# submission2019/cnn-quantization

Measured on NVIDIA H100. Metric: resnet50_w4a4_images_per_s, higher is better.
Workload: dtype f32

## Files before the change

cnn-quantization_b200/csrc/fq_cl.cuh:

```cuda
#pragma once

namespace fqb {

__device__ __forceinline__ unsigned enc_ordered(float x) {
  const unsigned b = __float_as_uint(x);
  return (b & 0x80000000u) ? ~b : (b | 0x80000000u);
}
__device__ __forceinline__ float dec_ordered(unsigned e) {
  return __uint_as_float((e & 0x80000000u) ? (e & 0x7fffffffu) : ~e);
}

constexpr unsigned kAccU = 2u * kMaxNhwcChannels;
constexpr unsigned kAccD = 3u * kMaxNhwcChannels;

struct ClView {
  unsigned* amin_inv;
  unsigned* amax;
  double* asum;
  double* asq;
  double* aabs;
};
__device__ __forceinline__ ClView cl_view(const FusedArgs& A, unsigned bank) {
  ClView v;
  v.amin_inv = A.amin_inv + bank * kAccU;
// ... 313 lines not shown
  T* st = reinterpret_cast<T*>(buf);
  consumer_sync();
#pragma unroll
  for (int i = 0; i < 4; ++i) st[i * kConsumers + threadIdx.x] = (threadIdx.x < stride) ? v[i] : identity;
  consumer_sync();
#pragma unroll
  for (unsigned k = 0; k < kClItems; ++k) {
    const unsigned it = threadIdx.x + k * kConsumers;
    T a = identity;
    if (it < 4u * cv) {
      const unsigned col = it % cv, i = it / cv;
      for (unsigned t = col; t < stride; t += cv) a = op(a, st[i * kConsumers + t]);
    }
    res[k] = a;
  }
}

__device__ __noinline__ void cl_combine_s1(unsigned char* buf, unsigned cv, unsigned stride, const unsigned (&umn)[4],
                                           const unsigned (&umx)[4], const double (&s)[4], const double (&q)[4], unsigned* dmn,
                                           unsigned* dmx, double* ds, double* dq) {
  if (cv == stride) {
    if (threadIdx.x < stride) {
#pragma unroll
      for (int i = 0; i < 4; ++i) {
        const unsigned c = 4u * threadIdx.x + i;
        red_max_u32(dmn + c, umn[i]);
        red_max_u32(dmx + c, umx[i]);
        red_add_f64(ds + c, s[i]);
        red_add_f64(dq + c, q[i]);
      }
    }
    return;
  }
  uint2 mm[4], rmm[kClItems];
#pragma unroll
  for (int i = 0; i < 4; ++i) mm[i] = make_uint2(umn[i], umx[i]);
  auto max2 = [](uint2 a, uint2 b) { return make_uint2(a.x > b.x ? a.x : b.x, a.y > b.y ? a.y : b.y); };
  double rs[kClItems], rq[kClItems];
  cl_stage_round(buf, cv, stride, mm, make_uint2(0u, 0u), max2, rmm);
  cl_stage_round(buf, cv, stride, s, 0.0, OpAdd(), rs);
  cl_stage_round(buf, cv, stride, q, 0.0, OpAdd(), rq);
#pragma unroll
  for (unsigned k = 0; k < kClItems; ++k) {
    const unsigned it = threadIdx.x + k * kConsumers;
    if (it < 4u * cv) {
      const unsigned c = 4u * (it % cv) + it / cv;
      red_max_u32(dmn + c, rmm[k].x);
      red_max_u32(dmx + c, rmm[k].y);
      red_add_f64(ds + c, rs[k]);
      red_add_f64(dq + c, rq[k]);
    }
  }
}
__device__ __noinline__ void cl_combine_add_f64(unsigned char* buf, unsigned cv, unsigned stride, const double (&v0)[4], double* d0,
                                                const double (&v1)[4], double* d1, const double (&v2)[4], double* d2) {
  if (cv == stride) {
    if (threadIdx.x < stride) {
#pragma unroll
      for (int i = 0; i < 4; ++i) {
        const unsigned c = 4u * threadIdx.x + i;
        red_add_f64(d0 + c, v0[i]);
        if (d1) red_add_f64(d1 + c, v1[i]);
        if (d2) red_add_f64(d2 + c, v2[i]);
      }
    }
    return;
  }
  double r0[kClItems], r1[kClItems], r2[kClItems];
  cl_stage_round(buf, cv, stride, v0, 0.0, OpAdd(), r0);
  if (d1) cl_stage_round(buf, cv, stride, v1, 0.0, OpAdd(), r1);
  if (d2) cl_stage_round(buf, cv, stride, v2, 0.0, OpAdd(), r2);
#pragma unroll
  for (unsigned k = 0; k < kClItems; ++k) {
    const unsigned it = threadIdx.x + k * kConsumers;
    if (it < 4u * cv) {
      const unsigned c = 4u * (it % cv) + it / cv;
      red_add_f64(d0 + c, r0[k]);
      if (d1) red_add_f64(d1 + c, r1[k]);
      if (d2) red_add_f64(d2 + c, r2[k]);
    }
  }
}

template <typename T, typename Op>
__device__ __forceinline__ T cl_rep_reduce(const T* p, unsigned rep, unsigned C, unsigned c, T identity, Op op) {
  T v[8];
#pragma unroll
  for (unsigned r = 0; r < 8u; ++r) v[r] = (r < rep) ? ld_ws(p + r * C + c) : identity;
  return op(op(op(v[0], v[1]), op(v[2], v[3])), op(op(v[4], v[5]), op(v[6], v[7])));
}
__device__ __forceinline__ double cl_mean(const ClView& acc, unsigned rep, unsigned C, unsigned c, float k, float bias, double n) {
  const double s = cl_rep_reduce(acc.asum, rep, C, c, 0.0, OpAdd());
  return static_cast<double>(k) + static_cast<double>(bias) + s / n;
}
__device__ __forceinline__ float cl_std(const ClView& acc, unsigned rep, unsigned C, unsigned c, double n) {
  const double s = cl_rep_reduce(acc.asum, rep, C, c, 0.0, OpAdd());
  const double q = cl_rep_reduce(acc.asq, rep, C, c, 0.0, OpAdd());
  double m2 = q - s * s / n;
  if (m2 < 0.0) m2 = 0.0;
  return static_cast<float>(sqrt(m2 / (n - 1.0)));
}

__device__ __forceinline__ LeafParam mid_tread_param(const FusedArgs& A, float omega, float mn, float mx, float mu, float b,
                                                     float& rng) {
  const bool sym = !A.positive;
  if (A.mt_clip) {
    double om = sym ? static_cast<double>(omega) : 2.0 * static_cast<double>(omega);
    int i = 0;
    while (i < kTable - 1 && kOmegaTable[i] < om) ++i;
    double am;
    if (i == 0) {
      am = kAlphaTable[0];
    } else {
      const double inc = (kAlphaTable[i] - kAlphaTable[i - 1]) / (kOmegaTable[i] - kOmegaTable[i - 1]);
      am = kAlphaTable[i] - inc * (kOmegaTable[i] - om);
    }
    const float amf = static_cast<float>(am);
    rng = sym ? __fmul_rn(__fmul_rn(2.f, amf), b) : __fadd_rn(fmaxf(mu, 0.f), __fmul_rn(amf, b));
  } else {
    rng = sym ? __fsub_rn(mx, mn) : mx;
  }
  const float step = (omega > 0.f) ? __fdiv_rn(rng, omega) : 3.402823466e+38f;
  LeafParam q;
  q.a = step;
  q.flags = 0;
  if (A.mt_clip) {
    const float mu_q = sym ? __fdiv_rn(mu, step) : __fdiv_rn(fmaxf(mu, 0.f), step);
    q.c = __fadd_rn(mu_q, sym ? __fmul_rn(omega, 0.5f) : omega);
    q.b = sym ? __fsub_rn(mu_q, __fmul_rn(omega, 0.5f)) : 0.f;
  } else {
    q.b = -INFINITY;
    q.c = INFINITY;
  }
  return q;
}

__device__ __noinline__ void cl_solve_aux(const FusedArgs& A, const ClView& acc, LeaderSmem& sm, unsigned tag, bool have_b,
                                          bool publish) {
  const unsigned C = A.flat.channels;
  const double n = A.n_per_group;
  const bool prior_b = (A.leaf != FQB200_LEAF_MIDTREAD) && A.prior == FQB200_PRIOR_B;
  for (unsigned c = threadIdx.x; c < C; c += kConsumers) {
    if (prior_b) {
      const double sa = have_b ? cl_rep_reduce(acc.aabs, A.nhwc_rep, C, c, 0.0, OpAdd()) : 0.0;
      A.gb[c] = static_cast<float>(sa / n);
    } else {
      A.gstd[c] = cl_std(acc, A.nhwc_rep, C, c, n);
    }
  }
  consumer_sync();
  stamp(A, 10);
  if (A.leaf == FQB200_LEAF_MIDTREAD) {
    double local = 0.0;
    for (unsigned c = threadIdx.x; c < C; c += kConsumers) {
      const float p = powf(A.gstd[c], 0.6666666666666666f);
      A.gprior[c] = p;
      local += static_cast<double>(p);
    }
    const float psum = static_cast<float>(block_reduce(local, OpAdd(), sm.d));
    const float budget = static_cast<float>(static_cast<double>(C) * exp2(static_cast<double>(A.mt_target)));
    for (unsigned c = threadIdx.x; c < C; c += kConsumers) A.gbits[c] = rintf(__fdiv_rn(__fmul_rn(budget, A.gprior[c]), psum));
  } else {
    solve_bit_alloc(A, sm);
  }
  consumer_sync();
  if (publish && threadIdx.x == 0) st_release_u32(&A.sync->aux_ready, tag);
}

template <int LEAF, bool DEV>
__device__ __noinline__ LeafParam cl_channel_param(const FusedArgs& A, const ClView& acc, unsigned rep, unsigned C, unsigned c,
                                                   float mu, double n, bool alloc, bool do_export) {
  auto umax = [](unsigned a, unsigned b) { return a > b ? a : b; };
  const unsigned lo = cl_rep_reduce(acc.amin_inv, rep, C, c, 0u, umax);
  const unsigned hi = cl_rep_reduce(acc.amax, rep, C, c, 0u, umax);
  const double sa = DEV ? cl_rep_reduce(acc.aabs, rep, C, c, 0.0, OpAdd()) : 0.0;
  const float cb = A.bias ? __ldg(A.bias + c) : 0.f;
  const float mn = __fadd_rn(dec_ordered(~lo), cb), mx = __fadd_rn(dec_ordered(hi), cb);
  const float b = DEV ? static_cast<float>(sa / n) : 0.f;
  const bool need_sd = A.range_mode == FQB200_RANGE_GAUS || A.range_mode == FQB200_RANGE_KSTD || do_export;
  const float sd = need_sd ? cl_std(acc, rep, C, c, n) : 0.f;
  const float aux = alloc ? ld_ws(A.gbits + c) : static_cast<float>(A.num_bits);
  LeafParam q;
  if constexpr (LEAF == FQB200_LEAF_MIDTREAD) {
    float rng;
    q = mid_tread_param(A, aux, mn, mx, mu, b, rng);
    if (do_export) export_stats(A, c, mn, mx, mu, b, sd, rng, 0.f, aux, q);
  } else {
    float delta, offset;
    solve_range(A, mn, mx, mu, b, sd, aux, delta, offset);
    q = make_leaf_param(LEAF, delta, offset, aux);
    if (do_export) export_stats(A, c, mn, mx, mu, b, sd, delta, offset, aux, q);
  }
  return q;
}

struct ClCtx {
  const FlatGeo* g;
  BulkRing* ring;
  unsigned char* stages;
  unsigned char* cbuf;
  RingPos pos;
  ClView acc;
  unsigned rep_base, c0;
  bool active;
};

__device__ __noinline__ void cl_phase_s1(const FusedArgs& A, ClCtx& cx, float (&kshift)[4]) {
  const FlatGeo& g = *cx.g;
  ClStats1 s1;
  s1.init(A, cx.c0, cx.active);
#pragma unroll
  for (int i = 0; i < 4; ++i) kshift[i] = s1.k[i];
  RingPos pos = cx.pos;
  consume_phase(g, *cx.ring, cx.stages, pos, s1);
  cx.pos = pos;
  s1.flush();
  if (blockIdx.x == 0) stamp(A, 13);
  unsigned umn[4], umx[4];
#pragma unroll
  for (int i = 0; i < 4; ++i) {
    umn[i] = ~enc_ordered(s1.mn[i]);
    umx[i] = enc_ordered(s1.mx[i]);
  }
  const ClView& acc = cx.acc;
  const unsigned rb = cx.rep_base;
  cl_combine_s1(cx.cbuf, g.cv, g.stride, umn, umx, s1.s, s1.q, acc.amin_inv + rb, acc.amax + rb, acc.asum + rb, acc.asq + rb);
}

__device__ __noinline__ void cl_phase_s2(const FusedArgs& A, ClCtx& cx, const float (&mean)[4]) {
  const FlatGeo& g = *cx.g;
  ClStats2 s2;
  s2.init(A, cx.c0, cx.active, mean);
  RingPos pos = cx.pos;
  consume_phase(g, *cx.ring, cx.stages, pos, s2);
  cx.pos = pos;
  s2.flush();
  if (blockIdx.x == 0) stamp(A, 14);
  const ClView& acc = cx.acc;
  const unsigned rb = cx.rep_base;
  cl_combine_add_f64(cx.cbuf, g.cv, g.stride, s2.sa, acc.aabs + rb, s2.sa, nullptr, s2.sa, nullptr);
}

template <int LEAF, bool HIST>
__device__ __noinline__ void cl_phase_apply(const FusedArgs& A, ClCtx& cx, const LeafParam (&lp)[4], unsigned* hist) {
  const FlatGeo& g = *cx.g;
  const unsigned t = threadIdx.x;
  if (HIST) {
    for (unsigned i = t; i < kHistWords; i += kConsumers) hist[i] = 0u;
    consumer_sync();
  }
  ClApply<LEAF, HIST> ap{A, hist};
  ap.init(cx.c0, cx.active, lp);
  RingPos pos = cx.pos;
  if (A.pool.tiles) {
    if (A.pool.kind == 3u)
      consume_pool3_phase(g, A.pool, *cx.ring, cx.stages, pos, ap);
    else
      consume_pool_phase(g, A.pool, *cx.ring, cx.stages, pos, ap);
  } else if (A.residual) {
    const FlatGeo h = half_geo(g);
    consume_pair_phase(h, *cx.ring, cx.stages, pos, ap);
  } else {
    consume_phase(g, *cx.ring, cx.stages, pos, ap);
  }
  cx.pos = pos;
  if (HIST) {
    consumer_sync();
    const unsigned bins = static_cast<unsigned>(A.hist_bins);
    const unsigned copies = max(1u, min(static_cast<unsigned>(kWarps), kHistWords / bins));
    for (unsigned b = t; b < bins; b += kConsumers) {
      unsigned long long cnt = 0;
      for (unsigned w = 0; w < copies; ++w) cnt += hist[w * bins + b];
      if (cnt) atomicAdd(A.hist + b, cnt);
    }
    if (LEAF == FQB200_LEAF_MIDTREAD && A.hist_clamped && cx.active) {
#pragma unroll
// ... 20 lines not shown
  __shared__ LeaderSmem lsm;
  __shared__ alignas(8) unsigned long long solver_done;
  const FlatGeo& g = A.flat;
  const unsigned C = g.channels, cv = g.cv;
  const unsigned launch = ld_ws(&A.sync->launch_count);
  const unsigned bank = launch & 1u;
  const unsigned tag = launch + 1u;
  const bool alloc = (LEAF == FQB200_LEAF_MIDTREAD) || (A.bit_alloc && A.num_bits <= 4);
  const bool aux_needs_b = alloc && LEAF != FQB200_LEAF_MIDTREAD && A.prior == FQB200_PRIOR_B;
  const bool solver_in_s2 = alloc && !aux_needs_b && DEV && gridDim.x > 1u;
  __shared__ alignas(8) unsigned long long phase_go[2];
  if (threadIdx.x == 0) {
    mbar_init(smem_u32(&solver_done), 1u);
    mbar_init(smem_u32(&phase_go[0]), 1u);
    mbar_init(smem_u32(&phase_go[1]), 1u);
  }
  const unsigned nstages = HIST ? kStages - 1u : kStages;
  ring_init(ring, nstages);

  if (threadIdx.x >= kConsumers) {
    if (threadIdx.x == kConsumers) {
      RingPos pos;
      pos.init(nstages);
      const float4* src = reinterpret_cast<const float4*>(A.in);
      const TicketPlan all = {2u, blockIdx.x, gridDim.x, 2u * gridDim.x};
      const TicketPlan no0 = {blockIdx.x == 0 ? 0u : 2u, blockIdx.x - 1u, gridDim.x - 1u, 2u * (gridDim.x - 1u)};
      produce_phase<false>(g, src, &A.sync->unit_counter[0], all, ring, stages, pos);
      if (DEV) {
        mbar_wait(smem_u32(&phase_go[0]), 0u);
        if (solver_in_s2 && blockIdx.x == 0) mbar_wait(smem_u32(&solver_done), 0u);
        produce_phase<true>(g, src, &A.sync->unit_counter[1], solver_in_s2 ? no0 : all, ring, stages, pos);
      }
      if (!A.stats_only) {
        mbar_wait(smem_u32(&phase_go[1]), 0u);
        if (A.pool.tiles && A.pool.kind == 3u)
          produce_pool3_phase(g, A.pool, src, &A.sync->unit_counter[2], all, ring, stages, pos);
        else if (A.pool.tiles)
          produce_pool_phase(g, A.pool, src, &A.sync->unit_counter[2], all, ring, stages, pos);
        else if (A.residual)
          produce_phase<!DEV, true>(half_geo(g), src, &A.sync->unit_counter[2], all, ring, stages, pos,
                                    reinterpret_cast<const float4*>(A.residual));
        else
          produce_phase<!DEV>(g, src, &A.sync->unit_counter[2], all, ring, stages, pos);
      }
    }
    return;
  }

  const unsigned t = threadIdx.x;
  const bool active = t < g.stride;
  const bool direct = cv == g.stride;
  const unsigned col = active ? t % cv : 0u;
  const unsigned c0 = 4u * col;
  const double n = A.n_per_group;
  const ClView acc = cl_view(A, bank);
  const unsigned rep = A.nhwc_rep;
  const unsigned rep_base = (blockIdx.x % rep) * C;
  unsigned epoch = 0;
  if (blockIdx.x == 0) stamp(A, 0);

  if (blockIdx.x == gridDim.x - 1u) {
    const ClView other = cl_view(A, bank ^ 1u);
    uint4* zu = reinterpret_cast<uint4*>(other.amin_inv);
    uint4* zd = reinterpret_cast<uint4*>(other.asum);
    const uint4 z = make_uint4(0u, 0u, 0u, 0u);
    for (unsigned i = t; i < kAccU / 4u; i += kConsumers) zu[i] = z;
    for (unsigned i = t; i < kAccD / 2u; i += kConsumers) zd[i] = z;
  }

  ClCtx cx;
  cx.g = &g;
  cx.ring = &ring;
  cx.stages = stages;
  cx.cbuf = cbuf;
  cx.pos.init(nstages);
  cx.acc = acc;
  cx.rep_base = rep_base;
  cx.c0 = c0;
  cx.active = active;
  float kshift[4];
  cl_phase_s1(A, cx, kshift);
  if (t == 0) mbar_arrive(smem_u32(&phase_go[DEV ? 0 : 1]));
  if (blockIdx.x == 0) stamp(A, 1);
  grid_barrier_cl(A.sync, epoch);
  if (blockIdx.x == 0) stamp(A, 4);

  float mean[4];
  if (direct) {
#pragma unroll
    for (int i = 0; i < 4; ++i)
      mean[i] = static_cast<float>(cl_mean(acc, rep, C, c0 + i, kshift[i], (A.bias && active) ? __ldg(A.bias + c0 + i) : 0.f, n));
  } else {
    for (unsigned c = t; c < C; c += kConsumers)
      tab_mean[c] = static_cast<float>(cl_mean(acc, rep, C, c, ld_tensor(A.in + c), A.bias ? __ldg(A.bias + c) : 0.f, n));
    consumer_sync();
#pragma unroll
    for (int i = 0; i < 4; ++i) mean[i] = tab_mean[c0 + i];
  }

  if (alloc && !aux_needs_b && blockIdx.x == 0) {
    cl_solve_aux(A, acc, lsm, tag, false, !solver_in_s2);
    stamp(A, 12);
    if (t == 0) mbar_arrive(smem_u32(&solver_done));
  }

  if constexpr (DEV) {
    cl_phase_s2(A, cx, mean);
    if (t == 0) mbar_arrive(smem_u32(&phase_go[1]));
    if (blockIdx.x == 0) stamp(A, 5);
    grid_barrier_cl(A.sync, epoch);
    if (blockIdx.x == 0) stamp(A, 8);
    if (aux_needs_b && blockIdx.x == 0) cl_solve_aux(A, acc, lsm, tag, true, true);
  }
  if (alloc && !solver_in_s2) {
    if (t == 0)
      while (ld_acquire_u32(&A.sync->aux_ready) != tag) __nanosleep(40);
    consumer_sync();
  }

  LeafParam lp[4];
  const bool do_export = A.out_stats != nullptr && blockIdx.x == 0;
  if (direct) {
#pragma unroll
    for (int i = 0; i < 4; ++i) lp[i] = cl_channel_param<LEAF, DEV>(A, acc, rep, C, c0 + i, mean[i], n, alloc, do_export && active);
  } else {
    LeafParam* tab_lp = reinterpret_cast<LeafParam*>(cbuf);
    consumer_sync();
    for (unsigned c = t; c < C; c += kConsumers) tab_lp[c] = cl_channel_param<LEAF, DEV>(A, acc, rep, C, c, tab_mean[c], n, alloc, do_export);
    consumer_sync();
#pragma unroll
    for (int i = 0; i < 4; ++i) lp[i] = tab_lp[c0 + i];
  }
  if (blockIdx.x == 0) stamp(A, 7);

  if (!A.stats_only) {
    cl_phase_apply<LEAF, HIST>(A, cx, lp, hist);
    if (blockIdx.x == 0) stamp(A, 9);
  }
  grid_exit_cl(A.sync);
}

template <bool GRID>
struct ClGiven {
  const FusedArgs& A;
  LeafParam q[4];
  float r[4], bias[4];
  bool fast;
  template <bool FAST>
  __device__ __forceinline__ void one(const float4& v, unsigned off) {
    const float x[4] = {v.x, v.y, v.z, v.w};
    float y[4], gq[4];
#pragma unroll
    for (int i = 0; i < 4; ++i) {
      Divisor dv;
      dv.s = q[i].a;
      dv.r = r[i];
      dv.fast = FAST;
      y[i] = leaf_apply<FQB200_LEAF_TORCH, FAST>(__fadd_rn(x[i], bias[i]), q[i], dv, 0.f, gq[i]);
    }
    st_tensor(reinterpret_cast<float4*>(A.out) + off, make_float4(y[0], y[1], y[2], y[3]));
    if (GRID) st_tensor(reinterpret_cast<float4*>(A.grid_out) + off, make_float4(gq[0], gq[1], gq[2], gq[3]));
  }
  __device__ __forceinline__ void consume(const float4& v, unsigned off) {
    if (fast)
      one<true>(v, off);
    else
      one<false>(v, off);
  }
  __device__ __forceinline__ void stage_end(const StageMeta&) {}
};

template <bool GRID>
__global__ void __launch_bounds__(kBulkThreads, kBulkCtasPerSm) fq_cl_given_kernel(const __grid_constant__ FusedArgs A) {
  extern __shared__ __align__(128) unsigned char fq_dyn[];
  __shared__ BulkRing ring;
  const FlatGeo& g = A.flat;
  ring_init(ring);
  if (threadIdx.x >= kConsumers) {
    if (threadIdx.x == kConsumers) {
      RingPos pos;
      pos.init();
      const TicketPlan tp = {0xffffffffu, blockIdx.x, gridDim.x, 0u};
      produce_phase<false>(g, reinterpret_cast<const float4*>(A.in), nullptr, tp, ring, fq_dyn, pos);
    }
    return;
  }
  const unsigned t = threadIdx.x;
  const bool active = t < g.stride;
  const unsigned c0 = active ? 4u * (t % g.cv) : 0u;
  ClGiven<GRID> ap{A};
  ap.fast = true;
#pragma unroll
  for (int i = 0; i < 4; ++i) {
    const unsigned c = c0 + i;
    const unsigned pi = A.given_per_group ? c : 0u;
    const float bits = A.g_bits ? __ldg(A.g_bits + c) : static_cast<float>(A.num_bits);
    ap.q[i] = make_leaf_param(FQB200_LEAF_TORCH, __ldg(A.g_delta + pi), __ldg(A.g_offset + pi), bits);
    const Divisor dv = make_divisor(ap.q[i].a);
    ap.r[i] = dv.r;
    ap.fast = ap.fast && dv.fast;
    ap.bias[i] = (A.bias && active) ? __ldg(A.bias + c) : 0.f;
  }
  RingPos pos;
  pos.init();
  consume_phase(g, ring, fq_dyn, pos, ap);
}

__global__ void __launch_bounds__(kBulkThreads, kBulkCtasPerSm) fq_cl_given_fused_kernel(const __grid_constant__ FusedArgs A) {
  extern __shared__ __align__(128) unsigned char fq_dyn[];
  __shared__ BulkRing ring;
  const FlatGeo& g = A.flat;
  ring_init(ring);
  if (threadIdx.x >= kConsumers) {
    if (threadIdx.x == kConsumers) {
      RingPos pos;
      pos.init();
      const float4* src = reinterpret_cast<const float4*>(A.in);
      const TicketPlan tp = {0xffffffffu, blockIdx.x, gridDim.x, 0u};
      if (A.pool.tiles && A.pool.kind == 3u)
        produce_pool3_phase(g, A.pool, src, nullptr, tp, ring, fq_dyn, pos);
      else if (A.pool.tiles)
// ... 387 lines not shown
  }
  __device__ __forceinline__ void pool_end(unsigned off) {
    float gq;
    float4 y;
    if (dv.fast) {
      y.x = leaf_apply<FQB200_LEAF_COMPILED, true>(__fadd_rn(pm[0], bias[0]), q, dv, 0.f, gq);
      y.y = leaf_apply<FQB200_LEAF_COMPILED, true>(__fadd_rn(pm[1], bias[1]), q, dv, 0.f, gq);
      y.z = leaf_apply<FQB200_LEAF_COMPILED, true>(__fadd_rn(pm[2], bias[2]), q, dv, 0.f, gq);
      y.w = leaf_apply<FQB200_LEAF_COMPILED, true>(__fadd_rn(pm[3], bias[3]), q, dv, 0.f, gq);
    } else {
      y.x = leaf_apply<FQB200_LEAF_COMPILED, false>(__fadd_rn(pm[0], bias[0]), q, dv, 0.f, gq);
      y.y = leaf_apply<FQB200_LEAF_COMPILED, false>(__fadd_rn(pm[1], bias[1]), q, dv, 0.f, gq);
      y.z = leaf_apply<FQB200_LEAF_COMPILED, false>(__fadd_rn(pm[2], bias[2]), q, dv, 0.f, gq);
      y.w = leaf_apply<FQB200_LEAF_COMPILED, false>(__fadd_rn(pm[3], bias[3]), q, dv, 0.f, gq);
    }
    st_tensor(reinterpret_cast<float4*>(A.pool_out) + off, y);
  }
  __device__ __forceinline__ void pooled(const float4& a0, const float4& a1, const float4& b0, const float4& b1, unsigned off) {
    pool_begin();
    pool_tap(a0);
    pool_tap(a1);
    pool_tap(b0);
    pool_tap(b1);
    pool_end(off);
  }
};

__global__ void __launch_bounds__(kBulkThreads, kBulkCtasPerSm) fq_rows_kernel(const __grid_constant__ FusedArgs A) {
  extern __shared__ __align__(128) unsigned char fq_dyn[];
  __shared__ BulkRing ring;
  __shared__ LeaderSmem lsm;
  __shared__ float scratch[2 * kWarps];
  const FlatGeo& g = A.flat;
  const RowsGeo& rg = A.rows;
  const unsigned bank = ld_ws(&A.sync->launch_count) & 1u;
  ring_init(ring);
  if (threadIdx.x >= kConsumers) {
    if (threadIdx.x == kConsumers) {
      RingPos pos;
      pos.init();
      const float4* src = reinterpret_cast<const float4*>(A.in);
      const TicketPlan all = {2u, blockIdx.x, gridDim.x, 2u * gridDim.x};
      produce_rows_phase<false>(g, rg, src, &A.sync->unit_counter[0], all, ring, fq_dyn, pos);
      if (!A.stats_only) {
        if (A.pool.tiles && A.pool.kind == 3u) {
          produce_pool3_phase(g, A.pool, src, &A.sync->unit_counter[2], all, ring, fq_dyn, pos);
        } else if (A.pool.tiles) {
          produce_pool_phase(g, A.pool, src, &A.sync->unit_counter[2], all, ring, fq_dyn, pos);
        } else if (A.residual) {
          const FlatGeo h = half_geo(g);
          produce_rows_phase<true, true>(h, half_rows(h, rg), src, &A.sync->unit_counter[2], all, ring, fq_dyn, pos,
                                         reinterpret_cast<const float4*>(A.residual));
        } else {
          produce_rows_phase<true>(g, rg, src, &A.sync->unit_counter[2], all, ring, fq_dyn, pos);
        }
      }
    }
    return;
  }
  const unsigned t = threadIdx.x;
  const bool active = t < g.stride;
  const unsigned c0 = active ? 4u * (t % g.cv) : 0u;
  const ClView acc = cl_view(A, bank);
  unsigned epoch = 0;
  RingPos pos;
  pos.init();
  if (blockIdx.x == 0) stamp(A, 0);
  if (blockIdx.x == gridDim.x - 1u) {
    const ClView other = cl_view(A, bank ^ 1u);
    uint4* zu = reinterpret_cast<uint4*>(other.amin_inv);
    uint4* zd = reinterpret_cast<uint4*>(other.asum);
    const uint4 z = make_uint4(0u, 0u, 0u, 0u);
    for (unsigned i = t; i < kAccU / 4u; i += kConsumers) zu[i] = z;
    for (unsigned i = t; i < kAccD / 2u; i += kConsumers) zd[i] = z;
  }
  float bias[4];
#pragma unroll
  for (int i = 0; i < 4; ++i) bias[i] = (A.bias && active) ? __ldg(A.bias + c0 + i) : 0.f;
  {
    RowsStats s1{A, scratch, acc, {bias[0], bias[1], bias[2], bias[3]}, INFINITY, -INFINITY};
    consume_phase(g, ring, fq_dyn, pos, s1);
  }
  if (blockIdx.x == 0) stamp(A, 1);
  grid_barrier_cl(A.sync, epoch);
  if (blockIdx.x == 0) stamp(A, 4);
  const unsigned R = rg.rows;
  float mn, mx;
  if (A.scope == FQB200_SCOPE_GROUP_MEAN) {
    double smin = 0.0, smax = 0.0;
    for (unsigned r = t; r < R; r += kConsumers) {
      smin += static_cast<double>(dec_ordered(~ld_ws(acc.amin_inv + r)));
      smax += static_cast<double>(dec_ordered(ld_ws(acc.amax + r)));
    }
    smin = block_reduce(smin, OpAdd(), lsm.d);
    smax = block_reduce(smax, OpAdd(), lsm.d);
    mn = static_cast<float>(smin / R);
    mx = static_cast<float>(smax / R);
  } else {
    float lmin = INFINITY, lmax = -INFINITY;
    for (unsigned r = t; r < R; r += kConsumers) {
      lmin = fminf(lmin, dec_ordered(~ld_ws(acc.amin_inv + r)));
      lmax = fmaxf(lmax, dec_ordered(ld_ws(acc.amax + r)));
    }
    mn = block_reduce(lmin, OpMin(), lsm.f);
    mx = block_reduce(lmax, OpMax(), lsm.f);
  }
  float delta, offset;
  solve_range(A, mn, mx, 0.f, 0.f, 0.f, static_cast<float>(A.num_bits), delta, offset);
  const LeafParam q = make_leaf_param(FQB200_LEAF_COMPILED, delta, offset, static_cast<float>(A.num_bits), A.relu_passthrough != 0);
  if (blockIdx.x == 0 && t == 0) export_stats(A, 0, mn, mx, 0.f, 0.f, 0.f, delta, offset, static_cast<float>(A.num_bits), q);
  if (blockIdx.x == 0) stamp(A, 7);
  if (!A.stats_only) {
    RowsApply ap{A, q, make_divisor(q.a), {bias[0], bias[1], bias[2], bias[3]}};
    ap.init_residual(c0, active);
    if (A.pool.tiles && A.pool.kind == 3u)
      consume_pool3_phase(g, A.pool, ring, fq_dyn, pos, ap);
    else if (A.pool.tiles)
      consume_pool_phase(g, A.pool, ring, fq_dyn, pos, ap);
    else if (A.residual)
      consume_pair_phase(half_geo(g), ring, fq_dyn, pos, ap);
    else
      consume_phase(g, ring, fq_dyn, pos, ap);
    if (blockIdx.x == 0) stamp(A, 9);
  }
  grid_exit_cl(A.sync);
}

}
```

cnn-quantization_b200/csrc/fqb200.cu:

```cuda
#include <cuda_runtime.h>
#include <math.h>
#include <stdint.h>
#include <stdio.h>
#include <stdlib.h>
#include <string.h>

#include "../../include/fqb200.h"
#include "fq_device.cuh"
#include "fq_bulk.cuh"

namespace fqb {

__constant__ float kGaus[9] = {0.f, 1.24f, 1.71f, 2.15f, 2.55f, 2.93f, 3.28f, 3.61f, 3.92f};
__constant__ float kGausPos[9] = {0.f, 1.71f, 2.15f, 2.55f, 2.93f, 3.28f, 3.61f, 3.92f, 4.2f};
__constant__ float kLaplace[9] = {1.05f, 1.86f, 2.83f, 3.89f, 5.03f, 6.2f, 7.41f, 8.64f, 9.89f};
__constant__ float kLaplacePos[9] = {1.86f, 2.83f, 3.89f, 5.02f, 6.2f, 7.41f, 8.64f, 9.89f, 11.16f};
constexpr int kTable = 101;
__constant__ double kOmegaTable[kTable];
__constant__ double kAlphaTable[kTable];

enum : int { FLAG_PASSTHROUGH = 1, FLAG_TRUE_ZERO = 2, FLAG_RELU = 4 };

struct alignas(16) LeafParam {
  float a, b, c;
  int flags;
};

struct FusedArgs {
  Geometry geo;
  FlatGeo flat;
  RowsGeo rows;
  const float* in;
  float* out;
  const float* residual;
  int residual_relu;
  PoolGeo pool;
  float* pool_out;
  const float* residual_stats;
  const float* residual_bias;
  const float* bias;
  unsigned long long bias_magic;
  float* grid_out;
  int scope, range_mode, leaf, num_bits, positive, solve_f64;
  float clip_k;
  int bit_alloc, prior, ba_round;
  float ba_target;
  float mt_target;
  int mt_clip;
  int bias_corr, var_corr, stats_only;
  int relu_passthrough;
  int need_dev;
  const float *g_delta, *g_offset, *g_bits;
  int given_per_group;
  unsigned inner;
  double n_per_group;
  float* out_stats;
  unsigned long long* hist_clamped;
  int hist_bins, hist_offset;
  unsigned long long* hist;
  unsigned long long* dbg;
  GridSync* sync;
  float *pmin, *pmax;
  double *psum, *pabs, *psq;
  float *gmin, *gmax, *gmean, *gb, *gstd, *gbits, *gprior;
  double* gmean_d;
  float *gdelta, *goffset;
  LeafParam* lp;
  float *cq, *co, *ck;
  unsigned *amin_inv, *amax;
  double *asum, *aabs, *asq;
  unsigned nhwc_rep;
};

constexpr unsigned kMaxNhwcChannels = 4096;

__device__ __forceinline__ void stamp(const FusedArgs& A, int slot) {
  if (A.dbg && threadIdx.x == 0) {
    unsigned long long t;
    asm volatile("mov.u64 %0, %globaltimer;" : "=l"(t));
    A.dbg[slot] = t;
  }
}

struct LeaderSmem {
  double d[kWarps];
  float f[kWarps];
  int i[kWarps];
  int flag;
};

template <typename T0, typename Op0, typename T1, typename Op1, typename T2, typename Op2>
__device__ __forceinline__ void reduce_partials3(const Geometry& geo, const T0* p0, T0* o0, T0 id0, Op0 op0, const T1* p1,
                                                 T1* o1, T1 id1, Op1 op1, const T2* p2, T2* o2, T2 id2, Op2 op2) {
  const unsigned L = geo.red_lanes;
  const unsigned sub = threadIdx.x % L;
  const unsigned per_sweep = kThreads / L;
  for (unsigned g0 = 0; g0 < geo.channels; g0 += per_sweep) {
    const unsigned g = g0 + threadIdx.x / L;
    T0 a0 = id0;
    T1 a1 = id1;
    T2 a2 = id2;
    if (g < geo.channels) {
#pragma unroll 4
      for (unsigned p = sub; p < geo.parts; p += L) {
        const size_t slot = static_cast<size_t>(p) * geo.channels + g;
        if (p0) a0 = op0(a0, ld_ws(p0 + slot));
        if (p1) a1 = op1(a1, ld_ws(p1 + slot));
        if (p2) a2 = op2(a2, ld_ws(p2 + slot));
      }
    }
    for (unsigned o = L >> 1; o > 0; o >>= 1) {
      a0 = op0(a0, __shfl_xor_sync(0xffffffffu, a0, o));
      a1 = op1(a1, __shfl_xor_sync(0xffffffffu, a1, o));
      a2 = op2(a2, __shfl_xor_sync(0xffffffffu, a2, o));
    }
    if (g < geo.channels && sub == 0) {
      if (p0) o0[g] = a0;
      if (p1) o1[g] = a1;
      if (p2) o2[g] = a2;
    }
  }
}

__device__ __noinline__ void solve_bit_alloc(const FusedArgs& A, LeaderSmem& sm) {
  const unsigned G = A.geo.channels;
  const float* prior = (A.prior == FQB200_PRIOR_STD) ? A.gstd : A.gb;
  constexpr unsigned kRegGroups = 4;
  const bool in_regs = G <= kRegGroups * kThreads;
  float pr[kRegGroups], bt[kRegGroups];
  double local = 0.0;
#pragma unroll
  for (unsigned k = 0; k < kRegGroups; ++k) {
    pr[k] = 0.f;
    bt[k] = 0.f;
  }
  if (in_regs) {
#pragma unroll
    for (unsigned k = 0; k < kRegGroups; ++k) {
      const unsigned g = threadIdx.x + k * kThreads;
      if (g < G) {
        pr[k] = powf(prior[g], 0.6666666666666666f);
        local += static_cast<double>(pr[k]);
      }
    }
  } else {
    for (unsigned g = threadIdx.x; g < G; g += kThreads) {
      float p = powf(prior[g], 0.6666666666666666f);
      A.gprior[g] = p;
      local += static_cast<double>(p);
    }
  }
  const float psum = static_cast<float>(block_reduce(local, OpAdd(), sm.d));
  stamp(A, 15);
  const float goal = A.ba_target;
  double m = static_cast<double>(A.ba_target);
  float half_gap = 1.0f;
  const float inv_g = 1.0f / static_cast<float>(G);
  int it = 0;
  __shared__ int warp_bits[2][kWarps];
  auto bits_of = [&](float p, float budget) {
    const float bins = __fdiv_rn(__fmul_rn(budget, p), psum);
    const float lg = log2f(bins);
    float bits = A.ba_round ? rintf(lg) : ceilf(lg);
    if (!(bits >= 0.f)) bits = 0.f;
    if (bits > 8.f) bits = 8.f;
    return bits;
  };
  while (fabsf(2.0f * half_gap) > 0.01f && it < 10) {
    const float budget = static_cast<float>(static_cast<double>(G) * exp2(m));
    int sum_bits = 0;
    if (in_regs) {
#pragma unroll
      for (unsigned k = 0; k < kRegGroups; ++k) {
        if (threadIdx.x + k * kThreads < G) {
          bt[k] = bits_of(pr[k], budget);
          sum_bits += static_cast<int>(bt[k]);
        }
      }
    } else {
      for (unsigned g = threadIdx.x; g < G; g += kThreads) {
        const float bits = bits_of(A.gprior[g], budget);
        A.gbits[g] = bits;
        sum_bits += static_cast<int>(bits);
      }
    }
    sum_bits = __reduce_add_sync(0xffffffffu, sum_bits);
    if ((threadIdx.x & 31) == 0) warp_bits[it & 1][threadIdx.x >> 5] = sum_bits;
    cta_sync();
    int total = 0;
#pragma unroll
    for (int w = 0; w < kWarps; ++w) total += warp_bits[it & 1][w];
    ++it;
    const float mean = __fmul_rn(static_cast<float>(total), inv_g);
    half_gap = __fmul_rn(__fsub_rn(goal, mean), 0.5f);
    m += static_cast<double>(half_gap);
  }
  stamp(A, 11);
  if (in_regs) {
#pragma unroll
    for (unsigned k = 0; k < kRegGroups; ++k) {
      const unsigned g = threadIdx.x + k * kThreads;
      if (g < G) A.gbits[g] = bt[k];
    }
  }
  cta_sync();
}

__device__ __forceinline__ void solve_range(const FusedArgs& A, float mn, float mx, float mean, float b, float sd,
                                            float bits, float& delta, float& offset) {
// ... 48 lines not shown
    q.flags = FLAG_TRUE_ZERO;
  } else {
    if (!(delta > 0.f)) {
      q.a = 1.f;
      q.b = 0.f;
      q.c = 0.f;
      q.flags = FLAG_PASSTHROUGH | (relu ? FLAG_RELU : 0);
      return q;
    }
    const float qmax = static_cast<float>((1 << static_cast<int>(bits)) - 1);
    const float scale = __fdiv_rn(delta, qmax);
    const bool tz = (__fadd_rn(offset, delta) > 0.f) && (offset < 0.f);
    q.a = scale;
    q.b = tz ? roundf(__fdiv_rn(-offset, scale)) : -offset;
    q.c = qmax;
    q.flags = tz ? FLAG_TRUE_ZERO : 0;
  }
  return q;
}

__device__ __forceinline__ void export_stats(const FusedArgs& A, unsigned g, float mn, float mx, float mean, float b,
                                             float sd, float delta, float offset, float bits, const LeafParam& q) {
  if (!A.out_stats) return;
  float* o = A.out_stats + static_cast<size_t>(g) * FQB200_STATS_STRIDE;
  o[0] = mn; o[1] = mx; o[2] = mean; o[3] = b; o[4] = sd; o[5] = delta; o[6] = offset; o[7] = bits;
  o[8] = q.a; o[9] = q.b; o[10] = q.c; o[11] = static_cast<float>(q.flags);
}

__device__ __noinline__ void solve_mid_tread(const FusedArgs& A, LeaderSmem& sm) {
  const unsigned G = A.geo.channels;
  double local = 0.0;
  for (unsigned g = threadIdx.x; g < G; g += kThreads) {
    float p = powf(A.gstd[g], 0.6666666666666666f);
    A.gprior[g] = p;
    local += static_cast<double>(p);
  }
  const float psum = static_cast<float>(block_reduce(local, OpAdd(), sm.d));
  const float budget = static_cast<float>(static_cast<double>(G) * exp2(static_cast<double>(A.mt_target)));
  const bool sym = !A.positive;
  for (unsigned g = threadIdx.x; g < G; g += kThreads) {
    const float omega = rintf(__fdiv_rn(__fmul_rn(budget, A.gprior[g]), psum));
    const float mn = A.gmin[g], mx = A.gmax[g], mu = A.gmean[g], b = A.gb[g];
    float rng;
    if (A.mt_clip) {
      double om = sym ? static_cast<double>(omega) : 2.0 * static_cast<double>(omega);
      int i = 0;
      while (i < kTable - 1 && kOmegaTable[i] < om) ++i;
      double am;
      if (i == 0) {
        am = kAlphaTable[0];
      } else {
        const double inc = (kAlphaTable[i] - kAlphaTable[i - 1]) / (kOmegaTable[i] - kOmegaTable[i - 1]);
        am = kAlphaTable[i] - inc * (kOmegaTable[i] - om);
      }
      const float amf = static_cast<float>(am);
      rng = sym ? __fmul_rn(__fmul_rn(2.f, amf), b) : __fadd_rn(fmaxf(mu, 0.f), __fmul_rn(amf, b));
    } else {
      rng = sym ? __fsub_rn(mx, mn) : mx;
    }
    const float step = (omega > 0.f) ? __fdiv_rn(rng, omega) : 3.402823466e+38f;
    LeafParam q;
    q.a = step;
    q.flags = 0;
    if (A.mt_clip) {
      const float mu_q = sym ? __fdiv_rn(mu, step) : __fdiv_rn(fmaxf(mu, 0.f), step);
      q.c = __fadd_rn(mu_q, sym ? __fmul_rn(omega, 0.5f) : omega);
      q.b = sym ? __fsub_rn(mu_q, __fmul_rn(omega, 0.5f)) : 0.f;
    } else {
      q.b = -INFINITY;
      q.c = INFINITY;
    }
    A.lp[g] = q;
    export_stats(A, g, mn, mx, mu, b, A.gstd[g], rng, 0.f, omega, q);
  }
}

__device__ __noinline__ void solve_params(const FusedArgs& A, LeaderSmem& sm) {
  const unsigned G = A.geo.channels;
  if (A.leaf == FQB200_LEAF_MIDTREAD) {
    solve_mid_tread(A, sm);
    return;
  }
  const bool alloc = A.bit_alloc && A.num_bits <= 4 && A.scope == FQB200_SCOPE_GROUP;
  if (alloc) solve_bit_alloc(A, sm);
  stamp(A, 12);
  if (A.scope != FQB200_SCOPE_GROUP) {
    float mn, mx;
    if (A.scope == FQB200_SCOPE_GROUP_MEAN) {
      double smin = 0.0, smax = 0.0;
      for (unsigned g = threadIdx.x; g < G; g += kThreads) {
        smin += static_cast<double>(A.gmin[g]);
        smax += static_cast<double>(A.gmax[g]);
      }
      smin = block_reduce(smin, OpAdd(), sm.d);
      smax = block_reduce(smax, OpAdd(), sm.d);
      mn = static_cast<float>(smin / G);
      mx = static_cast<float>(smax / G);
    } else {
      float lmin = INFINITY, lmax = -INFINITY;
      for (unsigned g = threadIdx.x; g < G; g += kThreads) {
        lmin = fminf(lmin, A.gmin[g]);
        lmax = fmaxf(lmax, A.gmax[g]);
      }
      mn = block_reduce(lmin, OpMin(), sm.f);
      mx = block_reduce(lmax, OpMax(), sm.f);
    }
    if (threadIdx.x == 0) {
      float delta, offset;
      solve_range(A, mn, mx, 0.f, 0.f, 0.f, static_cast<float>(A.num_bits), delta, offset);
      const LeafParam q = make_leaf_param(A.leaf, delta, offset, static_cast<float>(A.num_bits), A.relu_passthrough != 0);
      A.lp[0] = q;
      A.gdelta[0] = delta;
      A.goffset[0] = offset;
      export_stats(A, 0, mn, mx, 0.f, 0.f, 0.f, delta, offset, static_cast<float>(A.num_bits), q);
    }
    return;
  }
  for (unsigned g = threadIdx.x; g < G; g += kThreads) {
    const float bits = alloc ? A.gbits[g] : static_cast<float>(A.num_bits);
    const float mn = A.gmin[g], mx = A.gmax[g], mean = A.gmean[g];
    const float b = A.need_dev ? A.gb[g] : 0.f, sd = A.need_dev ? A.gstd[g] : 0.f;
    float delta, offset;
    solve_range(A, mn, mx, mean, b, sd, bits, delta, offset);
    const LeafParam q = make_leaf_param(A.leaf, delta, offset, bits, A.relu_passthrough != 0);
    A.lp[g] = q;
    A.gdelta[g] = delta;
    A.goffset[g] = offset;
    export_stats(A, g, mn, mx, mean, b, sd, delta, offset, bits, q);
  }
}

struct PhaseSmem {
  float f0[kWarps], f1[kWarps];
  double d0[kWarps], d1[kWarps];
  float bf0[4][kWarps], bf1[4][kWarps];
  double bd0[4][kWarps], bd1[4][kWarps];
  unsigned hist[kWarps][256];
};

__device__ __forceinline__ void hist_clear(PhaseSmem& sm) {
  for (unsigned i = threadIdx.x; i < kWarps * 256u; i += kThreads) (&sm.hist[0][0])[i] = 0u;
  cta_sync();
}
__device__ __forceinline__ void hist_add(PhaseSmem& sm, float q) {
  if (q >= 0.f && q <= 255.f) atomicAdd(&sm.hist[threadIdx.x >> 5][static_cast<unsigned>(q)], 1u);
}
__device__ __forceinline__ void hist_flush(PhaseSmem& sm, unsigned long long* out) {
  cta_sync();
  for (unsigned b = threadIdx.x; b < 256u; b += kThreads) {
    unsigned long long c = 0;
#pragma unroll
    for (int w = 0; w < kWarps; ++w) c += sm.hist[w][b];
    if (c) atomicAdd(out + b, c);
  }
}

#ifndef FQB_USTATS
#define FQB_USTATS 4
#endif
#ifndef FQB_UAPPLY
#define FQB_UAPPLY 4
#endif
__device__ __forceinline__ void block_combine(PhaseSmem& sm, float& mn, float& mx, double& s0, double& s1, bool use_f,
                                              bool use_d1) {
  if (use_f) {
    mn = warp_reduce(mn, OpMin());
    mx = warp_reduce(mx, OpMax());
// ... 1638 lines not shown
```

Before: 8908.

## Batch per-channel replica reductions and keep solver priors in shared staging

Result: no change. 8906, median of 6 (-0.0%).

```diff
diff --git a/cnn-quantization_b200/csrc/fq_cl.cuh b/cnn-quantization_b200/csrc/fq_cl.cuh
--- a/cnn-quantization_b200/csrc/fq_cl.cuh
+++ b/cnn-quantization_b200/csrc/fq_cl.cuh
@@ -419,23 +419,96 @@
   }
 }
 
+template <int J, int R, typename T, typename Op>
+__device__ __forceinline__ void cl_rep_reduce_n(const T* p, unsigned rep, unsigned C, unsigned c0, unsigned cstep, T identity, Op op,
+                                                T (&out)[J]) {
+  T v[J][8];
+#pragma unroll
+  for (int j = 0; j < J; ++j) {
+    const unsigned c = c0 + j * cstep;
+#pragma unroll
+    for (unsigned r = 0; r < 8u; ++r) v[j][r] = (r < static_cast<unsigned>(R) && r < rep && c < C) ? ld_ws(p + r * C + c) : identity;
+  }
+#pragma unroll
+  for (int j = 0; j < J; ++j)
+    out[j] = op(op(op(v[j][0], v[j][1]), op(v[j][2], v[j][3])), op(op(v[j][4], v[j][5]), op(v[j][6], v[j][7])));
+}
 template <typename T, typename Op>
 __device__ __forceinline__ T cl_rep_reduce(const T* p, unsigned rep, unsigned C, unsigned c, T identity, Op op) {
-  T v[8];
-#pragma unroll
-  for (unsigned r = 0; r < 8u; ++r) v[r] = (r < rep) ? ld_ws(p + r * C + c) : identity;
-  return op(op(op(v[0], v[1]), op(v[2], v[3])), op(op(v[4], v[5]), op(v[6], v[7])));
-}
-__device__ __forceinline__ double cl_mean(const ClView& acc, unsigned rep, unsigned C, unsigned c, float k, float bias, double n) {
-  const double s = cl_rep_reduce(acc.asum, rep, C, c, 0.0, OpAdd());
-  return static_cast<double>(k) + static_cast<double>(bias) + s / n;
+  T out[1];
+  cl_rep_reduce_n<1, 8>(p, rep, C, c, 0u, identity, op, out);
+  return out[0];
+}
+__device__ __forceinline__ int cl_batch(unsigned C, unsigned rep) {
+  if (C <= kConsumers) return 1;
+  if (C <= 2u * kConsumers && rep <= 4u) return 2;
+  if (C <= 3u * kConsumers && rep <= 3u) return 3;
+  if (C <= 4u * kConsumers && rep <= 2u) return 4;
+  return 0;
+}
+__device__ __forceinline__ float cl_mean_of(double s, float k, float bias, double n) {
+  return static_cast<float>(static_cast<double>(k) + static_cast<double>(bias) + s / n);
+}
+__device__ __forceinline__ float cl_std_of(double s, double q, double n) {
+  double m2 = q - s * s / n;
+  if (m2 < 0.0) m2 = 0.0;
+  return static_cast<float>(sqrt(m2 / (n - 1.0)));
 }
 __device__ __forceinline__ float cl_std(const ClView& acc, unsigned rep, unsigned C, unsigned c, double n) {
   const double s = cl_rep_reduce(acc.asum, rep, C, c, 0.0, OpAdd());
   const double q = cl_rep_reduce(acc.asq, rep, C, c, 0.0, OpAdd());
-  double m2 = q - s * s / n;
-  if (m2 < 0.0) m2 = 0.0;
-  return static_cast<float>(sqrt(m2 / (n - 1.0)));
+  return cl_std_of(s, q, n);
+}
+template <int J, int R>
+__device__ __forceinline__ void cl_means_n(const FusedArgs& A, const ClView& acc, unsigned rep, unsigned C, unsigned c0, unsigned cstep,
+                                           double n, float* tab) {
+  double s[J];
+  float k[J], cb[J];
+#pragma unroll
+  for (int j = 0; j < J; ++j) {
+    const unsigned c = c0 + j * cstep;
+    k[j] = c < C ? ld_tensor(A.in + c) : 0.f;
+    cb[j] = (A.bias && c < C) ? __ldg(A.bias + c) : 0.f;
+  }
+  cl_rep_reduce_n<J, R>(acc.asum, rep, C, c0, cstep, 0.0, OpAdd(), s);
+#pragma unroll
+  for (int j = 0; j < J; ++j)
+    if (c0 + j * cstep < C) tab[c0 + j * cstep] = cl_mean_of(s[j], k[j], cb[j], n);
+}
+template <int J, int R>
+__device__ __forceinline__ void cl_priors_n(const FusedArgs& A, const ClView& acc, unsigned rep, unsigned C, unsigned c0, unsigned cstep,
+                                            double n, bool prior_b, bool have_b, float* tab, float* mtab) {
+  if (prior_b) {
+    double sa[J];
+    if (have_b) {
+      cl_rep_reduce_n<J, R>(acc.aabs, rep, C, c0, cstep, 0.0, OpAdd(), sa);
+    } else {
+#pragma unroll
+      for (int j = 0; j < J; ++j) sa[j] = 0.0;
+    }
+#pragma unroll
+    for (int j = 0; j < J; ++j)
+      if (c0 + j * cstep < C) tab[c0 + j * cstep] = static_cast<float>(sa[j] / n);
+  } else {
+    double s[J], q[J];
+    float k[J], cb[J];
+#pragma unroll
+    for (int j = 0; j < J; ++j) {
+      const unsigned c = c0 + j * cstep;
+      k[j] = (mtab && c < C) ? ld_tensor(A.in + c) : 0.f;
+      cb[j] = (mtab && A.bias && c < C) ? __ldg(A.bias + c) : 0.f;
+    }
+    cl_rep_reduce_n<J, R>(acc.asum, rep, C, c0, cstep, 0.0, OpAdd(), s);
+    cl_rep_reduce_n<J, R>(acc.asq, rep, C, c0, cstep, 0.0, OpAdd(), q);
+#pragma unroll
+    for (int j = 0; j < J; ++j) {
+      const unsigned c = c0 + j * cstep;
+      if (c < C) {
+        tab[c] = cl_std_of(s[j], q[j], n);
+        if (mtab) mtab[c] = cl_mean_of(s[j], k[j], cb[j], n);
+      }
+    }
+  }
 }
 
 __device__ __forceinline__ LeafParam mid_tread_param(const FusedArgs& A, float omega, float mn, float mx, float mu, float b,
@@ -473,32 +546,31 @@
 }
 
 __device__ __noinline__ void cl_solve_aux(const FusedArgs& A, const ClView& acc, LeaderSmem& sm, unsigned tag, bool have_b,
-                                          bool publish) {
-  const unsigned C = A.flat.channels;
+                                          bool publish, float* pri, float* mtab) {
+  const unsigned C = A.flat.channels, rep = A.nhwc_rep, t = threadIdx.x;
   const double n = A.n_per_group;
   const bool prior_b = (A.leaf != FQB200_LEAF_MIDTREAD) && A.prior == FQB200_PRIOR_B;
-  for (unsigned c = threadIdx.x; c < C; c += kConsumers) {
-    if (prior_b) {
-      const double sa = have_b ? cl_rep_reduce(acc.aabs, A.nhwc_rep, C, c, 0.0, OpAdd()) : 0.0;
-      A.gb[c] = static_cast<float>(sa / n);
-    } else {
-      A.gstd[c] = cl_std(acc, A.nhwc_rep, C, c, n);
-    }
+  switch (cl_batch(C, rep)) {
+    case 2: cl_priors_n<2, 4>(A, acc, rep, C, t, kConsumers, n, prior_b, have_b, pri, mtab); break;
+    case 3: cl_priors_n<3, 3>(A, acc, rep, C, t, kConsumers, n, prior_b, have_b, pri, mtab); break;
+    case 4: cl_priors_n<4, 2>(A, acc, rep, C, t, kConsumers, n, prior_b, have_b, pri, mtab); break;
+    default:
+      for (unsigned c = t; c < C; c += kConsumers) cl_priors_n<1, 8>(A, acc, rep, C, c, 0u, n, prior_b, have_b, pri, mtab);
   }
   consumer_sync();
   stamp(A, 10);
   if (A.leaf == FQB200_LEAF_MIDTREAD) {
     double local = 0.0;
     for (unsigned c = threadIdx.x; c < C; c += kConsumers) {
-      const float p = powf(A.gstd[c], 0.6666666666666666f);
-      A.gprior[c] = p;
+      const float p = powf(pri[c], 0.6666666666666666f);
+      pri[c] = p;
       local += static_cast<double>(p);
     }
     const float psum = static_cast<float>(block_reduce(local, OpAdd(), sm.d));
     const float budget = static_cast<float>(static_cast<double>(C) * exp2(static_cast<double>(A.mt_target)));
-    for (unsigned c = threadIdx.x; c < C; c += kConsumers) A.gbits[c] = rintf(__fdiv_rn(__fmul_rn(budget, A.gprior[c]), psum));
+    for (unsigned c = threadIdx.x; c < C; c += kConsumers) A.gbits[c] = rintf(__fdiv_rn(__fmul_rn(budget, pri[c]), psum));
   } else {
-    solve_bit_alloc(A, sm);
+    solve_bit_alloc(A, sm, pri);
   }
   consumer_sync();
   if (publish && threadIdx.x == 0) st_release_u32(&A.sync->aux_ready, tag);
@@ -506,17 +578,12 @@
 
 template <int LEAF, bool DEV>
 __device__ __noinline__ LeafParam cl_channel_param(const FusedArgs& A, const ClView& acc, unsigned rep, unsigned C, unsigned c,
-                                                   float mu, double n, bool alloc, bool do_export) {
-  auto umax = [](unsigned a, unsigned b) { return a > b ? a : b; };
-  const unsigned lo = cl_rep_reduce(acc.amin_inv, rep, C, c, 0u, umax);
-  const unsigned hi = cl_rep_reduce(acc.amax, rep, C, c, 0u, umax);
-  const double sa = DEV ? cl_rep_reduce(acc.aabs, rep, C, c, 0.0, OpAdd()) : 0.0;
-  const float cb = A.bias ? __ldg(A.bias + c) : 0.f;
+                                                   float mu, double n, bool do_export, unsigned lo, unsigned hi, double sa, float aux,
+                                                   float cb) {
   const float mn = __fadd_rn(dec_ordered(~lo), cb), mx = __fadd_rn(dec_ordered(hi), cb);
   const float b = DEV ? static_cast<float>(sa / n) : 0.f;
   const bool need_sd = A.range_mode == FQB200_RANGE_GAUS || A.range_mode == FQB200_RANGE_KSTD || do_export;
   const float sd = need_sd ? cl_std(acc, rep, C, c, n) : 0.f;
-  const float aux = alloc ? ld_ws(A.gbits + c) : static_cast<float>(A.num_bits);
   LeafParam q;
   if constexpr (LEAF == FQB200_LEAF_MIDTREAD) {
     float rng;
@@ -529,6 +596,35 @@
     if (do_export) export_stats(A, c, mn, mx, mu, b, sd, delta, offset, aux, q);
   }
   return q;
+}
+template <int LEAF, bool DEV, int J, int R>
+__device__ __forceinline__ void cl_channel_params(const FusedArgs& A, const ClView& acc, unsigned rep, unsigned C, unsigned c0,
+                                                  unsigned cstep, const float (&mu)[J], double n, bool alloc, bool do_export,
+                                                  LeafParam (&q)[J]) {
+  auto umax = [](unsigned a, unsigned b) { return a > b ? a : b; };
+  unsigned lo[J], hi[J];
+  double sa[J];
+  float aux[J], cb[J];
+#pragma unroll
+  for (int j = 0; j < J; ++j) cb[j] = (A.bias && c0 + j * cstep < C) ? __ldg(A.bias + c0 + j * cstep) : 0.f;
+  cl_rep_reduce_n<J, R>(acc.amin_inv, rep, C, c0, cstep, 0u, umax, lo);
+  cl_rep_reduce_n<J, R>(acc.amax, rep, C, c0, cstep, 0u, umax, hi);
+  if (DEV) {
+    cl_rep_reduce_n<J, R>(acc.aabs, rep, C, c0, cstep, 0.0, OpAdd(), sa);
+  } else {
+#pragma unroll
+    for (int j = 0; j < J; ++j) sa[j] = 0.0;
+  }
+#pragma unroll
+  for (int j = 0; j < J; ++j) {
+    const unsigned c = c0 + j * cstep;
+    aux[j] = (alloc && c < C) ? ld_ws(A.gbits + c) : static_cast<float>(A.num_bits);
+  }
+#pragma unroll
+  for (int j = 0; j < J; ++j) {
+    const unsigned c = c0 + j * cstep;
+    if (c < C) q[j] = cl_channel_param<LEAF, DEV>(A, acc, rep, C, c, mu[j], n, do_export, lo[j], hi[j], sa[j], aux[j], cb[j]);
+  }
 }
 
 struct ClCtx {
@@ -715,35 +811,47 @@
   cl_phase_s1(A, cx, kshift);
   if (t == 0) mbar_arrive(smem_u32(&phase_go[DEV ? 0 : 1]));
   if (blockIdx.x == 0) stamp(A, 1);
+  stamp_last(A, 2);
   grid_barrier_cl(A.sync, epoch);
   if (blockIdx.x == 0) stamp(A, 4);
 
   float mean[4];
-  if (direct) {
-#pragma unroll
-    for (int i = 0; i < 4; ++i)
-      mean[i] = static_cast<float>(cl_mean(acc, rep, C, c0 + i, kshift[i], (A.bias && active) ? __ldg(A.bias + c0 + i) : 0.f, n));
-  } else {
-    for (unsigned c = t; c < C; c += kConsumers)
-      tab_mean[c] = static_cast<float>(cl_mean(acc, rep, C, c, ld_tensor(A.in + c), A.bias ? __ldg(A.bias + c) : 0.f, n));
-    consumer_sync();
-#pragma unroll
-    for (int i = 0; i < 4; ++i) mean[i] = tab_mean[c0 + i];
-  }
-
-  if (alloc && !aux_needs_b && blockIdx.x == 0) {
-    cl_solve_aux(A, acc, lsm, tag, false, !solver_in_s2);
+  const bool solver = alloc && !aux_needs_b && blockIdx.x == 0;
+  if (solver) {
+    static_assert(kClStagingBytes / 8u >= 4u * kConsumers, "prior and mean tables of C <= 2048 channels fit the staging");
+    float* pri = reinterpret_cast<float*>(cbuf);
+    float* mtab = direct ? pri + kClStagingBytes / 8u : tab_mean;
+    cl_solve_aux(A, acc, lsm, tag, false, !solver_in_s2, pri, mtab);
     stamp(A, 12);
     if (t == 0) mbar_arrive(smem_u32(&solver_done));
+#pragma unroll
+    for (int i = 0; i < 4; ++i) mean[i] = mtab[c0 + i];
+  } else if (direct) {
+    double s[4];
+    float cb[4];
+#pragma unroll
+    for (int i = 0; i < 4; ++i) cb[i] = (A.bias && active) ? __ldg(A.bias + c0 + i) : 0.f;
+    cl_rep_reduce_n<4, 3>(acc.asum, rep, C, c0, 1u, 0.0, OpAdd(), s);
+#pragma unroll
+    for (int i = 0; i < 4; ++i) mean[i] = cl_mean_of(s[i], kshift[i], cb[i], n);
+  } else {
+    if (cl_batch(C, rep) == 2)
+      cl_means_n<2, 4>(A, acc, rep, C, t, kConsumers, n, tab_mean);
+    else
+      for (unsigned c = t; c < C; c += kConsumers) cl_means_n<1, 8>(A, acc, rep, C, c, 0u, n, tab_mean);
+    consumer_sync();
+#pragma unroll
+    for (int i = 0; i < 4; ++i) mean[i] = tab_mean[c0 + i];
   }
 
   if constexpr (DEV) {
     cl_phase_s2(A, cx, mean);
     if (t == 0) mbar_arrive(smem_u32(&phase_go[1]));
     if (blockIdx.x == 0) stamp(A, 5);
+    stamp_last(A, 3);
     grid_barrier_cl(A.sync, epoch);
     if (blockIdx.x == 0) stamp(A, 8);
-    if (aux_needs_b && blockIdx.x == 0) cl_solve_aux(A, acc, lsm, tag, true, true);
+    if (aux_needs_b && blockIdx.x == 0) cl_solve_aux(A, acc, lsm, tag, true, true, reinterpret_cast<float*>(cbuf), nullptr);
   }
   if (alloc && !solver_in_s2) {
     if (t == 0)
@@ -754,12 +862,25 @@
   LeafParam lp[4];
   const bool do_export = A.out_stats != nullptr && blockIdx.x == 0;
   if (direct) {
-#pragma unroll
-    for (int i = 0; i < 4; ++i) lp[i] = cl_channel_param<LEAF, DEV>(A, acc, rep, C, c0 + i, mean[i], n, alloc, do_export && active);
+    cl_channel_params<LEAF, DEV, 4, 3>(A, acc, rep, C, c0, 1u, mean, n, alloc, do_export && active, lp);
   } else {
     LeafParam* tab_lp = reinterpret_cast<LeafParam*>(cbuf);
     consumer_sync();
-    for (unsigned c = t; c < C; c += kConsumers) tab_lp[c] = cl_channel_param<LEAF, DEV>(A, acc, rep, C, c, tab_mean[c], n, alloc, do_export);
+    if (cl_batch(C, rep) == 2) {
+      const unsigned c1 = t + kConsumers;
+      const float mu[2] = {tab_mean[t], c1 < C ? tab_mean[c1] : 0.f};
+      LeafParam q[2];
+      cl_channel_params<LEAF, DEV, 2, 4>(A, acc, rep, C, t, kConsumers, mu, n, alloc, do_export, q);
+      tab_lp[t] = q[0];
+      if (c1 < C) tab_lp[c1] = q[1];
+    } else {
+      for (unsigned c = t; c < C; c += kConsumers) {
+        const float mu[1] = {tab_mean[c]};
+        LeafParam q[1];
+        cl_channel_params<LEAF, DEV, 1, 8>(A, acc, rep, C, c, 0u, mu, n, alloc, do_export, q);
+        tab_lp[c] = q[0];
+      }
+    }
     consumer_sync();
 #pragma unroll
     for (int i = 0; i < 4; ++i) lp[i] = tab_lp[c0 + i];
@@ -770,6 +891,7 @@
     cl_phase_apply<LEAF, HIST>(A, cx, lp, hist);
     if (blockIdx.x == 0) stamp(A, 9);
   }
+  stamp_last(A, 6);
   grid_exit_cl(A.sync);
 }
 
@@ -1323,6 +1445,7 @@
     consume_phase(g, ring, fq_dyn, pos, s1);
   }
   if (blockIdx.x == 0) stamp(A, 1);
+  stamp_last(A, 2);
   grid_barrier_cl(A.sync, epoch);
   if (blockIdx.x == 0) stamp(A, 4);
   const unsigned R = rg.rows;
@@ -1364,6 +1487,7 @@
       consume_phase(g, ring, fq_dyn, pos, ap);
     if (blockIdx.x == 0) stamp(A, 9);
   }
+  stamp_last(A, 6);
   grid_exit_cl(A.sync);
 }
 
diff --git a/cnn-quantization_b200/csrc/fqb200.cu b/cnn-quantization_b200/csrc/fqb200.cu
--- a/cnn-quantization_b200/csrc/fqb200.cu
+++ b/cnn-quantization_b200/csrc/fqb200.cu
@@ -81,6 +81,13 @@
     A.dbg[slot] = t;
   }
 }
+__device__ __forceinline__ void stamp_last(const FusedArgs& A, int slot) {
+  if (A.dbg && threadIdx.x == 0) {
+    unsigned long long t;
+    asm volatile("mov.u64 %0, %globaltimer;" : "=l"(t));
+    atomicMax(A.dbg + slot, ((t & ((1ull << 52) - 1ull)) << 12) | blockIdx.x);
+  }
+}
 
 struct LeaderSmem {
   double d[kWarps];
@@ -122,9 +129,8 @@
   }
 }
 
-__device__ __noinline__ void solve_bit_alloc(const FusedArgs& A, LeaderSmem& sm) {
+__device__ __noinline__ void solve_bit_alloc(const FusedArgs& A, LeaderSmem& sm, const float* prior) {
   const unsigned G = A.geo.channels;
-  const float* prior = (A.prior == FQB200_PRIOR_STD) ? A.gstd : A.gb;
   constexpr unsigned kRegGroups = 4;
   const bool in_regs = G <= kRegGroups * kThreads;
   float pr[kRegGroups], bt[kRegGroups];
@@ -339,7 +345,7 @@
     return;
   }
   const bool alloc = A.bit_alloc && A.num_bits <= 4 && A.scope == FQB200_SCOPE_GROUP;
-  if (alloc) solve_bit_alloc(A, sm);
+  if (alloc) solve_bit_alloc(A, sm, A.prior == FQB200_PRIOR_STD ? A.gstd : A.gb);
   stamp(A, 12);
   if (A.scope != FQB200_SCOPE_GROUP) {
     float mn, mx;
```
